# Healthcare-Robotics/assistive-vr-gym

Hardware: AMD Instinct MI355X
Metric: env-steps/sec at N parallel envs, 1/2/4/8 MI355X; max |dq| vs PyBullet (higher is better)
Workload: dtype f32; 1 GPU; FeedingJaco-v0, 4096 envs/GPU, rigid-only, random actions; task=FeedingJaco-v0, envs_per_gpu=4096, impairment=random, parallelism=env-sharded x1, env_groups=4, stepping=rollout

## Files before the change

### assistive-vr-gym_amd/csrc/avr_kernel.hip

```cpp
#include <hip/hip_runtime.h>
#include <stdint.h>

#include "../../include/avr.h"
#include <cstring>
#include <cstdlib>
#include "avr_math.h"

#include "avr_kmodel.h"

typedef float f2v __attribute__((ext_vector_type(2)));
typedef float f4v __attribute__((ext_vector_type(4)));
typedef __attribute__((address_space(3))) float lds_f;
#define AVR_GA __attribute__((address_space(1)))
template <class T> __device__ __forceinline__ T gld(const T *p) { return *(const AVR_GA T *)p; }
__device__ __forceinline__ int2 gld(const int2 *p) { const AVR_GA int *q = (const AVR_GA int *)p; return make_int2(q[0], q[1]); }
__device__ __forceinline__ float2 gld(const float2 *p) { const f2v x = *(const AVR_GA f2v *)p; return make_float2(x.x, x.y); }
__device__ __forceinline__ float4 gld(const float4 *p) { const f4v x = *(const AVR_GA f4v *)p; return make_float4(x.x, x.y, x.z, x.w); }
__device__ __forceinline__ v3 gld3(const float *p) { const AVR_GA float *q = (const AVR_GA float *)p; return V(q[0], q[1], q[2]); }
__device__ __forceinline__ qt gldq(const float *p) { const AVR_GA float *q = (const AVR_GA float *)p; return Q(q[0], q[1], q[2], q[3]); }
__device__ __forceinline__ tf gldtf(const float *p) { tf r; r.p = gld3(p); r.q = gldq(p + 3); return r; }
typedef __attribute__((address_space(3))) f2v lds_f2;
typedef __attribute__((address_space(3))) f4v lds_f4;
typedef __attribute__((address_space(3))) int lds_i;
typedef const __attribute__((address_space(1))) float *gfp;
// ... 3253 lines not shown
    pcount(33, T);
#endif
    for (int c0 = 0; c0 < T; c0 += 64) {
#ifdef AVR_PROF
        int pit = 0, pk = -1;
#endif
        if (c0 + lane < T) {
            float *cs;
            (void)item(c0 + lane, cs);
            const int2 e = entry(c0 + lane);
            const float *bt = btfs[slot_of(c0 + lane)];
            const int k = e.x & 0xffff;
            const int sa = e.y & 0xffff, sb = e.y >> 16;
            const int ba = (e.x >> 16) & 0xff, bb = (e.x >> 24) & 0xff;
            const int vrow = cs_vrow(m, cs), vbo = vrow * m.nb, vso = vrow * m.ns;
            const float thr = fminf(gld(m.body_threshold + (vbo + ba)), gld(m.body_threshold + (vbo + bb)));
            const WShape A = make_wshape(m, sa, ldtf(bt + 8 * ba), vso), B = make_wshape(m, sb, ldtf(bt + 8 * bb), vso);
            int rc = 2;
            v3 nB = V(0, 0, 0), pB = V(0, 0, 0);
            float d = 0.f;
            if (!((A.nv > SMALL_NV && A.tab < 0) || (B.nv > SMALL_NV && B.tab < 0))) {
                int nit, nkind;
                rc = narrowphase<false>(m, *(EpaBuf *)cs, A, B, thr, nB, pB, d, nit, nkind);
#ifdef AVR_PROF
                pit = nit; pk = nkind;
#endif
            }
            np_store(cs, k, rc, nB, pB, d);
        }
#ifdef AVR_PROF
        int mx = pit;
        for (int o = 32; o; o >>= 1) mx = max(mx, __shfl_xor(mx, o));
        int sm = pit;
        for (int o = 32; o; o >>= 1) sm += __shfl_xor(sm, o);
        pcount(36, sm);
        pcount(37, mx);
        pcount(38, __popcll(__ballot(pk == 3)));
        pcount(39, __popcll(__ballot(pk >= 0 && pk < 3)));
#endif
    }
}

__global__ __launch_bounds__(64) __attribute__((amdgpu_waves_per_eu(NP_WAVES))) void avr_narrowphase_kernel(const KModel *__restrict__ mp, const unsigned char *__restrict__ mask, int env0,
                                                             int n_envs) {
    const int list = (blockIdx.x >> 3) & 1;
    const int eb = env0 + 8 * NP_ENVS * (blockIdx.x >> 4) + (blockIdx.x & 7);
    if (eb >= n_envs) return;
    __shared__ float2 ent[NP_ENVS * MAXSP];
    __shared__ float btfs[NP_ENVS][MAXB * 8];
    np_list(*mp, mask, eb, list, n_envs, ent, btfs);
}

#ifndef AVR_COOP_KERNEL
#define AVR_COOP_KERNEL 0
#endif
#if AVR_COOP_KERNEL
__global__ __launch_bounds__(64) void avr_coop_kernel(const KModel *__restrict__ mp, const unsigned char *__restrict__ mask, int env0, int n_envs) {
    __shared__ EpaBuf E;
    AVR_ENV_GUARD();
    if (gld(env_cs(m, env) + CS_COOP) != 0.f) {
        float *ws = env_ws(m, env);
        const int rot = __float_as_int(gld(ws + WS_COOPROT));
        (void)np_coop(m, env_cs(m, env), __float_as_int(gld(env_cs(m, env) + CS_NSP)), E, rot, 1 << 30);
        if (lane_id() == 0) ws[WS_COOPROT] = __int_as_float(rot + AVR_COOP_CAP);
    }
}
#endif

AVR_DI void substep_a_env(const KModel &m, EnvLDS &L, float *__restrict__ state, float dt, int env, int n_envs) {
    (void)n_envs;
    WT_START();
    static_assert(sizeof(EpaBuf) <= sizeof(EnvLDS), "EPA buffer overlay");
#if !AVR_COOP_KERNEL
    float *gst = state + (size_t)env * K_STATE_WORDS;
    const bool persist = gld(gst + S_TASK + T_COOPN) >= (float)AVR_COOP_PERSIST;
    int demand = 0;
    if (gld(env_cs(m, env) + CS_COOP) != 0.f) {
        float *ws = env_ws(m, env);
        const int rot = __float_as_int(gld(ws + WS_COOPROT));
        demand = np_coop(m, env_cs(m, env), __float_as_int(gld(env_cs(m, env) + CS_NSP)), *reinterpret_cast<EpaBuf *>(&L), rot,
                         persist ? AVR_COOP_CAP : 1 << 30);
        if (lane_id() == 0) ws[WS_COOPROT] = __int_as_float(rot + AVR_COOP_CAP);
        SYNC();
    }
#endif
#if AVR_COOP_KERNEL
    float *gst = state + (size_t)env * K_STATE_WORDS;
#endif
    load_a(m, L, gst, env_cs(m, env));
#if !AVR_COOP_KERNEL
    if (lane_id() == 0) {
        L.st[S_TASK + T_COOPN] = demand > AVR_COOP_CAP ? L.st[S_TASK + T_COOPN] + 1.f : 0.f;
        if (persist && demand > AVR_COOP_CAP) L.flags |= 32;
    }
    SYNC();
#endif
    bool ok = substep_a(m, L, dt, gst, env_ws(m, env), env_rows(m, env), env_cs(m, env), K_DYN_ROLE ? env_dynho(m, env) : nullptr);
#ifdef AVR_PROF
    if (lane_id() == 0) env_ws(m, env)[WS_XCC] = __int_as_float(xcc_id());
#endif
    if (lane_id() == 0 && !ok) L.flags |= 1;
    SYNC();
    if (lane_id() == 0) L.st[S_TASK + T_FLAGS] = (float)((int)L.st[S_TASK + T_FLAGS] | L.flags);
    SYNC();
    if (lane_id() < 16) gst[S_TASK + lane_id()] = L.st[S_TASK + lane_id()];
    prof_flush(m, L, env);
    WT_END(0);
}

__global__ __launch_bounds__(64) AVR_KATTR void avr_substep_a_kernel(const KModel *__restrict__ mp, float *__restrict__ state,
                                                                     const unsigned char *__restrict__ mask, float dt, int env0, int n_envs) {
    __shared__ EnvLDS L;
    AVR_ENV_GUARD();
    substep_a_env(m, L, state, dt, env, n_envs);
}

#if B4_PK
struct DV { float rq, rq2; f2v v1, v2, v3; };
#else
struct DV { float rq, rq2, vx, vy, vz, wx, wy, wz; };
#endif

AVR_DI int uni(int x) { return __builtin_amdgcn_readfirstlane(x); }

#define B4_OOB 0x7fff0000
typedef __amdgpu_buffer_rsrc_t rsrc_t;
typedef unsigned u4v __attribute__((ext_vector_type(4)));
typedef unsigned u3v __attribute__((ext_vector_type(3)));
typedef unsigned u2v __attribute__((ext_vector_type(2)));
AVR_DI f4v bld4(rsrc_t r, int o) { u4v x = __builtin_amdgcn_raw_buffer_load_b128(r, o, 0, 0); return *(f4v *)&x; }
AVR_DI f2v bld2(rsrc_t r, int o) { u2v x = __builtin_amdgcn_raw_buffer_load_b64(r, o, 0, 0); return *(f2v *)&x; }
AVR_DI float bld1(rsrc_t r, int o) { return __uint_as_float(__builtin_amdgcn_raw_buffer_load_b32(r, o, 0, 0)); }
#if NDL == 2
typedef f4v rv_t;
#define RVB 16
#define rload bld4
#else
typedef f2v rv_t;
#define RVB 8
#define rload bld2
#endif
typedef __attribute__((address_space(3))) rv_t lds_rv;
AVR_DI f4v bld3(rsrc_t r, int o) {
    u3v x = __builtin_amdgcn_raw_buffer_load_b96(r, o, 0, 0);
    f4v y = {__uint_as_float(x.x), __uint_as_float(x.y), __uint_as_float(x.z), 0.f};
    return y;
}

#ifndef B4_LDSW
#define B4_LDSW 10240
#endif
AVR_DI int al4(int x) { return (x + 3) & ~3; }

AVR_DI int own_of(int mask) {
    const int sl = lane_id() & 15;
    return (int)__builtin_amdgcn_ubfe((unsigned)mask, sl < MAXF ? 2 * sl : 30, 2);
}
static_assert(2 * MAXF <= CI_SLOT && MAXNC + K_CROWS * K_MAX_CONTACTS < (1 << (30 - CI_SLOT)), "own mask and slot bit fields");


struct NcRow { int o; lds_f *ip; f4v h0, h1; float imp; f2v j0, j1, j2; rv_t r; };
struct NcSrc {
    typedef NcRow Row;
    static constexpr bool robot_parts = true;
    rsrc_t rs;
    int eo, ro;
    lds_f *ip0, *nullip;
    AVR_DI void set(Row &R, bool v, int o, lds_f *ip) const { R.o = v ? o : B4_OOB; R.ip = v ? ip : nullip; }
    AVR_DI void hdr(Row &R) const { R.h0 = bld4(rs, R.o); R.h1 = bld3(rs, R.o + 16); R.imp = *R.ip; }
    AVR_DI void parts(Row &R) const {
        const int o = own_of(__float_as_int(R.h0.x));
        const int b = o ? R.o + 8 + 24 * o : B4_OOB;
        R.j0 = bld2(rs, b); R.j1 = bld2(rs, b + 8); R.j2 = bld2(rs, b + 16);
        const int slot = __float_as_int(R.h0.y) - 1;
        R.r = rload(rs, slot >= 0 ? ro + slot * (ROBW * 4) + RVB * (lane_id() & 15) : B4_OOB);
    }
};

#define LN_HEAD (NDL == 2 ? 80 : 48)
#define LNB_NULL 24
#define LNB_ZERO 48
#define LNB_NCNULL 16
typedef __attribute__((address_space(3))) char lds_c;
struct NcLds {
    typedef NcRow Row;
    static constexpr bool robot_parts = true;
    lds_c *blk;
    int eo;
    unsigned rob;
    lds_f *ip0, *nullip;
    AVR_DI void set(Row &R, bool v, int o, lds_f *ip) const { R.o = v ? o : LNB_NCNULL; R.ip = v ? ip : nullip; }
    AVR_DI void hdr(Row &R) const {
        R.h0 = *(const lds_f4 *)(blk + R.o - 8);
        const f2v a = *(const lds_f2 *)(blk + R.o + 8);
        R.h1.x = a.x; R.h1.y = a.y; R.h1.z = *(const lds_f *)(blk + R.o + 16);
        R.imp = *R.ip;
    }
    AVR_DI void parts(Row &R) const {
        const int w = own_of(__float_as_int(R.h0.x));
        const lds_f2 *q = (const lds_f2 *)(blk + (w ? R.o + 24 * w : LNB_ZERO));
        R.j0 = q[0]; R.j1 = q[1]; R.j2 = q[2];
        const unsigned sp = (unsigned)__float_as_int(R.h0.y);
        R.r = *(const lds_rv *)(blk + (sp ? rob + ROBW * 4 * sp : LNB_ZERO));
    }
};

struct CRowL { unsigned wb; lds_f *ip; f4v h; float imp; f2v j0, j1, j2; rv_t r; };
template <bool RC>
struct CLds {
    typedef CRowL Row;
    static constexpr bool robot_parts = RC;
    lds_c *blk;
    unsigned cn, cf;
    unsigned rob;
    lds_f *ipn, *ipf, *nullip;
    unsigned ct;
    lds_f *ipt;
    AVR_DI void set(Row &R, bool v, unsigned wb, lds_f *ip) const { R.wb = v ? wb : LNB_NULL; R.ip = v ? ip : nullip; }
    AVR_DI void hdr(Row &R) const { R.h = *(const lds_f4 *)(blk + R.wb + 8); R.imp = *R.ip; }
    AVR_DI void hdr3(Row &R) const {
        const lds_f *q = (const lds_f *)(blk + R.wb + 8);
        const f2v a = *(const lds_f2 *)q;
        R.h.x = a.x; R.h.y = a.y; R.h.z = q[2];
        R.imp = *R.ip;
    }
    AVR_DI void hdr2(Row &B, const Row &A) const {
        B.h = *(const lds_f4 *)(blk + A.wb + 8 + CRW * 4);
        B.imp = A.ip[1];
    }
    AVR_DI unsigned own_b(const Row &R) const { const int o = own_of(__float_as_int(R.h.x)); return o ? R.wb + 24 * o : LNB_ZERO; }
    AVR_DI void own_at(Row &R, unsigned b) const { const lds_f2 *q = (const lds_f2 *)(blk + b); R.j0 = q[0]; R.j1 = q[1]; R.j2 = q[2]; }
    AVR_DI unsigned rob_b(const Row &R) const { const unsigned s = (unsigned)__float_as_int(R.h.x) >> CI_SLOT; return s ? rob + ROBW * 4 * s : LNB_ZERO; }
    AVR_DI rv_t rob_at(unsigned b) const {
        if constexpr (!RC) { (void)b; return rv_t{}; }
        return *(const lds_rv *)(blk + b);
    }
    AVR_DI void parts(Row &R) const { own_at(R, own_b(R)); R.r = rob_at(rob_b(R)); }
    AVR_DI int tor_of(int c) const { return (int)((unsigned)__float_as_int(*(const lds_f *)(blk + cn + CRW * 4 * c + 8)) >> 2 & 0x3ffffu); }
    AVR_DI void unit_parts(Row &A, Row &B) const {
        const unsigned b = own_b(A), r = rob_b(A);
        own_at(A, b); own_at(B, b + CRW * 4);
        A.r = rob_at(r); B.r = rob_at(r + ROBW * 4);
    }
};

struct CRowG { int o; lds_f *ip; f4v h; float imp; f2v j0, j1, j2; rv_t r; };
struct CGlb {
    typedef CRowG Row;
    static constexpr bool robot_parts = true;
    rsrc_t rs;
    int cn, cf;
    int rob;
    lds_f *ipn, *ipf, *nullip;
    int ct;
    lds_f *ipt;
    AVR_DI void set(Row &R, bool v, int o, lds_f *ip) const { R.o = v ? o : B4_OOB; R.ip = v ? ip : nullip; }
    AVR_DI void hdr(Row &R) const { R.h = bld4(rs, R.o); R.imp = *R.ip; }
    AVR_DI void hdr3(Row &R) const { R.h = bld3(rs, R.o); R.imp = *R.ip; }
    AVR_DI void hdr2(Row &B, const Row &A) const { B.h = bld4(rs, A.o + CRW * 4); B.imp = A.ip[1]; }
    AVR_DI int own_b(const Row &R) const { const int o = own_of(__float_as_int(R.h.x)); return o ? R.o - 8 + 24 * o : B4_OOB; }
    AVR_DI void own_at(Row &R, int b) const { R.j0 = bld2(rs, b); R.j1 = bld2(rs, b + 8); R.j2 = bld2(rs, b + 16); }
    AVR_DI int rob_b(const Row &R) const { const int s = (int)((unsigned)__float_as_int(R.h.x) >> CI_SLOT); return s ? rob + ROBW * 4 * s : B4_OOB; }
    AVR_DI rv_t rob_at(int b) const { return rload(rs, b); }
    AVR_DI void parts(Row &R) const { own_at(R, own_b(R)); R.r = rob_at(rob_b(R)); }
    AVR_DI int tor_of(int c) const { return (int)((unsigned)__float_as_int(bld1(rs, cn + CRW * 4 * c)) >> 2 & 0x3ffffu); }
    AVR_DI void unit_parts(Row &A, Row &B) const {
        const int b = own_b(A), r = rob_b(A);
        own_at(A, b); own_at(B, b + CRW * 4);
        A.r = rob_at(r); B.r = rob_at(r + ROBW * 4);
    }
};

AVR_DI float row16_sum(float x) {
    x += __int_as_float(__builtin_amdgcn_update_dpp(0, __float_as_int(x), 0x128, 0xf, 0xf, true));
    x += __int_as_float(__builtin_amdgcn_update_dpp(0, __float_as_int(x), 0x124, 0xf, 0xf, true));
    x += __int_as_float(__builtin_amdgcn_update_dpp(0, __float_as_int(x), 0x122, 0xf, 0xf, true));
    x += __int_as_float(__builtin_amdgcn_update_dpp(0, __float_as_int(x), 0x121, 0xf, 0xf, true));
    return x;
}

template <bool RP, class R>
AVR_DI float go4(const R &X, DV &d, float imp, float inv, float rhs, float lo, float hi, float rl = 0.f, unsigned long long *acc = nullptr) {
#pragma clang fp contract(off)
#if B4_PK
    f2v s = X.j0 * d.v1;
    if (RP) {
        s.y = fmaf(X.r.x, d.rq, s.y);
#if NDL == 2
        s.y = fmaf(X.r.z, d.rq2, s.y);
#endif
    }
    s = __builtin_elementwise_fma(X.j1, d.v2, s);
    s = __builtin_elementwise_fma(X.j2, d.v3, s);
    const float dv = row16_sum(s.x + s.y);
    const float ni = __builtin_amdgcn_fmed3f(imp + fmaf(-dv, inv, rhs), lo, hi);
    const float delta = ni - imp;
    if (acc) *acc |= __ballot(fabsf(delta) > rl);
    const f2v dd = {delta, delta};
    d.v1 = __builtin_elementwise_fma(X.j0, dd, d.v1);
    d.v2 = __builtin_elementwise_fma(X.j1, dd, d.v2);
    d.v3 = __builtin_elementwise_fma(X.j2, dd, d.v3);
    if (RP) d.rq = fmaf(X.r.y, delta, d.rq);
#if NDL == 2
    if (RP) d.rq2 = fmaf(X.r.w, delta, d.rq2);
#endif
    return ni;
#else
    const float p = fmaf(X.j1.x, d.vz, fmaf(X.j0.y, d.vy, X.j0.x * d.vx));
#if NDL == 2
    const float q = RP ? fmaf(X.j2.y, d.wz, fmaf(X.j2.x, d.wy, fmaf(X.r.z, d.rq2, fmaf(X.r.x, d.rq, X.j1.y * d.wx))))
                       : fmaf(X.j2.y, d.wz, fmaf(X.j2.x, d.wy, X.j1.y * d.wx));
#else
    const float q = RP ? fmaf(X.j2.y, d.wz, fmaf(X.j2.x, d.wy, fmaf(X.r.x, d.rq, X.j1.y * d.wx)))
                       : fmaf(X.j2.y, d.wz, fmaf(X.j2.x, d.wy, X.j1.y * d.wx));
#endif
    const float dv = row16_sum(p + q);
    const float ni = __builtin_amdgcn_fmed3f(imp + fmaf(-dv, inv, rhs), lo, hi);
    const float delta = ni - imp;
    if (acc) *acc |= __ballot(fabsf(delta) > rl);
    d.vx = fmaf(X.j0.x, delta, d.vx); d.vy = fmaf(X.j0.y, delta, d.vy); d.vz = fmaf(X.j1.x, delta, d.vz);
    d.wx = fmaf(X.j1.y, delta, d.wx); d.wy = fmaf(X.j2.x, delta, d.wy); d.wz = fmaf(X.j2.y, delta, d.wz);
    if (RP) d.rq = fmaf(X.r.y, delta, d.rq);
#if NDL == 2
    if (RP) d.rq2 = fmaf(X.r.w, delta, d.rq2);
#endif
    return ni;
#endif
}

#if B4_FPAIR
template <bool RP, class R>
AVR_DI void go4_pair(const R &A, const R &B, DV &d, float &ia, float &ib, float lim) {
#pragma clang fp contract(off)
    f2v sa = A.j0 * d.v1, sb = B.j0 * d.v1;
    if (RP) {
        sa.y = fmaf(A.r.x, d.rq, sa.y); sb.y = fmaf(B.r.x, d.rq, sb.y);
#if NDL == 2
        sa.y = fmaf(A.r.z, d.rq2, sa.y); sb.y = fmaf(B.r.z, d.rq2, sb.y);
#endif
    }
    sa = __builtin_elementwise_fma(A.j1, d.v2, sa); sb = __builtin_elementwise_fma(B.j1, d.v2, sb);
    sa = __builtin_elementwise_fma(A.j2, d.v3, sa); sb = __builtin_elementwise_fma(B.j2, d.v3, sb);
    const float dva = row16_sum(sa.x + sa.y), dvb0 = row16_sum(sb.x + sb.y);
    const float na = __builtin_amdgcn_fmed3f(ia + fmaf(-dva, A.h.y, A.h.z), -lim, lim);
    const float da = na - ia;
    const float dvb = fmaf(da, B.h.w, dvb0);
    const float nb = __builtin_amdgcn_fmed3f(ib + fmaf(-dvb, B.h.y, B.h.z), -lim, lim);
    const float db = nb - ib;
    const f2v dda = {da, da}, ddb = {db, db};
    d.v1 = __builtin_elementwise_fma(B.j0, ddb, __builtin_elementwise_fma(A.j0, dda, d.v1));
    d.v2 = __builtin_elementwise_fma(B.j1, ddb, __builtin_elementwise_fma(A.j1, dda, d.v2));
    d.v3 = __builtin_elementwise_fma(B.j2, ddb, __builtin_elementwise_fma(A.j2, dda, d.v3));
    if (RP) d.rq = fmaf(B.r.y, db, fmaf(A.r.y, da, d.rq));
#if NDL == 2
    if (RP) d.rq2 = fmaf(B.r.w, db, fmaf(A.r.w, da, d.rq2));
#endif
    ia = na; ib = nb;
}
#endif

template <int D, bool H3, class S>
AVR_DI void hdr_of(const S &s, typename S::Row &R) {
    if constexpr (H3) s.hdr3(R);
    else s.hdr(R);
}
template <int D, bool H3, class S, class AT, class GO>
AVR_DI void sweep4(const S &s, int n, const AT &at, const GO &go) {
    if (n <= 0) return;
    constexpr int K = 2 * D + 1;
    typename S::Row R[K];
#pragma unroll
    for (int q = 0; q < 2 * D; q++) { at(R[q], q); hdr_of<D, H3>(s, R[q]); }
#pragma unroll
    for (int q = 0; q < D; q++) s.parts(R[q]);
    for (int j = 0; j < n; j += K) {
#pragma unroll
        for (int q = 0; q < K; q++) {
            at(R[(q + 2 * D) % K], j + q + 2 * D);
            hdr_of<D, H3>(s, R[(q + 2 * D) % K]);
            s.parts(R[(q + D) % K]);
            go(R[q]);
        }
    }
}

template <class S>
struct Pair4 { typename S::Row a, b; float in; };

#if K_TORSION
template <class CS>
struct TorRow : CS::Row { float in; };
template <class CS>
struct TorSrc {
    typedef TorRow<CS> Row;
    static constexpr bool robot_parts = CS::robot_parts;
    const CS &cs;
    AVR_DI void hdr(Row &R) const { cs.hdr(R); }
    AVR_DI void parts(Row &R) const { cs.parts(R); }
};
#endif

AVR_DI int wave_max4(int x) {
    x = max(x, __shfl_xor(x, 16));
    x = max(x, __shfl_xor(x, 32));
    return uni(x);
}

template <int DN, int DC, class NS, class CS>
AVR_DI int pgs4(const KModel &m, const NS &ns, const CS &cs, lds_i *list, lds_i *tlist, int n_nc, int n_c, int nnc_max, int nc_max, DV &d) {
    typedef typename NS::Row NR;
    typedef typename CS::Row CR;
    const int sl = lane_id() & 15;
#if B4_PK
    d.rq = d.rq2 = 0.f; d.v1 = d.v2 = d.v3 = f2v{0.f, 0.f};
#else
    d.rq = d.rq2 = 0.f; d.vx = d.vy = d.vz = d.wx = d.wy = d.wz = 0.f;
#endif
    auto at_n = [&](CR &R, int j) { cs.set(R, j < n_c, cs.cn + CRW * 4 * j, cs.ipn + j); };
    sweep4<DC, true>(cs, nc_max, at_n, [&](const CR &R) { (void)go4<CS::robot_parts>(R, d, 0.f, R.h.y, R.h.z, R.imp, R.imp); });
    int units = 0;
    bool done = false;
    for (int it = 0; it < m.iters; it++) {
        const int a_nc = done ? 0 : n_nc, a_c = done ? 0 : n_c;
        const int anc_max = wave_max4(a_nc), ac_max = wave_max4(a_c);
        unsigned long long acc = 0ull;
        const bool fwd = (it & 1) != 0;
        const int r0 = fwd ? 0 : n_nc - 1, sg = fwd ? 1 : -1;
        const int ob = ns.eo + r0 * (RWC * 4);
        lds_f *ib = ns.ip0 + r0;
        sweep4<DN, false>(ns, anc_max, [&](NR &R, int j) { ns.set(R, j < a_nc, ob + sg * j * (RWC * 4), ib + sg * j); },
                          [&](const NR &R) { *R.ip = go4<true>(R, d, R.imp, R.h0.z, R.h0.w, R.h1.x, R.h1.y, R.h1.z, &acc); });
        auto at_na = [&](CR &R, int j) { cs.set(R, j < a_c, cs.cn + CRW * 4 * j, cs.ipn + j); };
        sweep4<DC, false>(cs, ac_max, at_na, [&](const CR &R) { *R.ip = go4<CS::robot_parts>(R, d, R.imp, R.h.y, R.h.z, 0.f, 1e10f, R.h.w, &acc); });
        int t = 0;
        for (int c0 = 0; c0 < ac_max; c0 += 16) {
            const int c = c0 + sl;
            const bool a = c < a_c && cs.ipn[c < a_c ? c : 0] > 0.f;
            const unsigned long long b = __ballot(a);
            const unsigned gm = (unsigned)(b >> (lane_id() & 48)) & 0xffffu;
            if (a) list[t + __popc(gm & ((1u << sl) - 1u))] = c;
            t += __popc(gm);
        }
        const int tmax = wave_max4(t);
        units += tmax;
        if (tmax > 0) {
        constexpr int K = 2 * DC + 1;
        Pair4<CS> X[K];
        auto lst = [&](int u) { const int c = list[u < t ? u : 0]; return u < t ? c : -1; };
        auto hdr = [&](Pair4<CS> &Y, int c) {
            cs.set(Y.a, c >= 0, cs.cf + 2 * CRW * 4 * c, cs.ipf + 2 * c);
            cs.hdr(Y.a);
            cs.hdr2(Y.b, Y.a);
            const float x = cs.ipn[max(c, 0)];
            Y.in = c >= 0 ? x : 0.f;
        };
        auto go = [&](const Pair4<CS> &Y) {
            const float lim = Y.a.h.w * Y.in;
#if B4_FPAIR
            float ia = Y.a.imp, ib = Y.b.imp;
            go4_pair<CS::robot_parts>(Y.a, Y.b, d, ia, ib, lim);
            Y.a.ip[0] = ia; Y.a.ip[1] = ib;
#else
            Y.a.ip[0] = go4<CS::robot_parts>(Y.a, d, Y.a.imp, Y.a.h.y, Y.a.h.z, -lim, lim, Y.b.h.x, &acc);
            Y.a.ip[1] = go4<CS::robot_parts>(Y.b, d, Y.b.imp, Y.b.h.y, Y.b.h.z, -lim, lim, Y.b.h.w, &acc);
#endif
        };
        int cn = lst(0);
#pragma unroll
        for (int q = 0; q < 2 * DC; q++) { hdr(X[q], cn); cn = lst(q + 1); }
#pragma unroll
        for (int q = 0; q < DC; q++) cs.unit_parts(X[q].a, X[q].b);
        for (int u0 = 0; u0 < tmax; u0 += K) {
#pragma unroll
            for (int q = 0; q < K; q++) {
                hdr(X[(q + 2 * DC) % K], cn);
                cn = lst(u0 + q + 2 * DC + 1);
                cs.unit_parts(X[(q + DC) % K].a, X[(q + DC) % K].b);
                go(X[q]);
            }
        }
#if K_TORSION
        {
            int tt = 0;
            for (int u0 = 0; u0 < tmax; u0 += 16) {
                const int u = u0 + sl;
                const int cl = list[u < t ? u : 0];
                const int c = u < t ? cl : 0;
                const int tv = cs.tor_of(c);
                const bool a = u < t && tv > 0;
                const unsigned long long b = __ballot(a);
                const unsigned gm = (unsigned)(b >> (lane_id() & 48)) & 0xffffu;
                if (a) tlist[tt + __popc(gm & ((1u << sl) - 1u))] = c | (tv - 1) << 8;
                tt += __popc(gm);
            }
            int ttmax = tt;
            ttmax = max(ttmax, __shfl_xor(ttmax, 16));
            ttmax = max(ttmax, __shfl_xor(ttmax, 32));
            ttmax = uni(ttmax);
            const TorSrc<CS> ts{cs};
            sweep4<DC, false>(ts, 3 * ttmax, [&](TorRow<CS> &R, int j) {
                const int u = j / 3, k = j - 3 * u;
                const bool v = u < tt;
                const int e = tlist[v ? u : 0];
                const int c = e & 255, ti = e >> 8;
                cs.set(R, v, cs.ct + 3 * CRW * 4 * ti + CRW * 4 * k, cs.ipt + 3 * ti + k);
                const float x = cs.ipn[v ? c : 0];
                R.in = v ? x : 0.f;
            }, [&](const TorRow<CS> &R) {
                const float lim = R.h.w * R.in;
                *R.ip = go4<CS::robot_parts>(R, d, R.imp, R.h.y, R.h.z, -lim, lim, BT_RESIDUAL_SQRT * R.h.y, &acc);
            });
        }
#endif
        }
        done = done || ((acc >> (lane_id() & 48)) & 0xffffull) == 0ull;
        if (__ballot(!done) == 0ull) break;
    }
    return units;
}

#ifndef B4_DN
#define B4_DN 2
#endif
#ifndef B4_DC
#define B4_DC 1
#endif
#ifndef B4_DG
#define B4_DG 3
#endif
#ifndef B4_NC_LDS
#define B4_NC_LDS K_PR2
#endif
#ifndef B4_DNL
#define B4_DNL 1
#endif

#ifndef B4_SORT
#define B4_SORT 0
#endif
AVR_DI int b4_env(const KModel &m, const unsigned char *__restrict__ mask, int env0, int n_envs, int bidx, int g) {
    const int x = bidx & 7, j = bidx >> 3;
#if B4_SORT
    const int lane = lane_id();
    const int kc = (j >> 5) << 7;
    unsigned key[2];
#pragma unroll
    for (int h = 0; h < 2; h++) {
        const int kk = lane + 64 * h;
        const int e = env0 + x + 8 * (kc + kk);
        unsigned cost = 0xffffffu;
        if (e < n_envs) {
            cost = 0u;
            if (!mask || mask[e]) {
                const float *ws = env_ws(m, e);
                cost = (unsigned)(__float_as_int(gld(ws + WS_NNC)) + 3 * __float_as_int(gld(ws + WS_NC)) +
                                  (K_TORSION ? 3 * __float_as_int(gld(ws + WS_NT)) : 0));
                cost = min(cost, 0xfffffeu);
            }
        }
        key[h] = (cost << 7) | (unsigned)kk;
    }
    int rank0 = 0, rank1 = 0;
    for (int i = 0; i < 64; i++) {
        const unsigned a = __builtin_amdgcn_readlane(key[0], i), b = __builtin_amdgcn_readlane(key[1], i);
        rank0 += (a < key[0]) + (b < key[0]);
        rank1 += (a < key[1]) + (b < key[1]);
    }
    int pick = 0;
#pragma unroll
    for (int gg = 0; gg < 4; gg++) {
        const int r = 4 * (j & 31) + gg;
        const unsigned long long b0 = __ballot(rank0 == r), b1 = __ballot(rank1 == r);
        const int kk = b0 ? __builtin_ctzll(b0) : 64 + __builtin_ctzll(b1);
        if (g == gg) pick = kk;
    }
    return env0 + x + 8 * (kc + pick);
#else
    (void)m; (void)mask; (void)n_envs;
    return env0 + 32 * j + x + 8 * g;
#endif
}

AVR_DI void substep_b4_block(const KModel &m, float *__restrict__ state, const unsigned char *__restrict__ mask, float dt, int frame_end,
                             int env0, int n_envs, int bidx, lds_f *blk) {
#ifdef AVR_WAVETIME
    const unsigned long long wt0 = __builtin_amdgcn_s_memrealtime();
#endif
    const int lane = lane_id(), sl = lane & 15, g = lane >> 4;
    const int env = b4_env(m, mask, env0, n_envs, bidx, g);
    const bool live = env < n_envs && (!mask || mask[env]);
    const int ev = live ? env : env0;
    const gfp wsg = (gfp)env_ws(m, ev);
    float *st = state + (size_t)ev * K_STATE_WORDS;
    const int n_nc = live ? __float_as_int(wsg[WS_NNC]) : 0, n_c = live ? __float_as_int(wsg[WS_NC]) : 0;
    const int n_rob = live ? __float_as_int(wsg[WS_NROB]) : 0;
    const int n_t = live && K_TORSION ? __float_as_int(wsg[WS_NT]) : 0;
    const int n_cr = 3 * n_c + 3 * n_t;
    const int n_rows = n_nc + n_cr, n_rc = max(n_rob - n_nc, 0);
    auto wmax = [&](int x) { x = max(x, __shfl_xor(x, 16)); x = max(x, __shfl_xor(x, 32)); return uni(x); };
    const int nnc_max = wmax(n_nc), nc_max = wmax(n_c);
    const rsrc_t rs = __builtin_amdgcn_make_buffer_rsrc(m.rows, 0, m.rows_envs * m.rowstride * 4, 0x00020000);
    const int eo = ev * m.rowstride * 4, ro = eo + m.rowcap * RWC * 4;
#ifdef AVR_LDS_POISON
    for (int i = lane; i < B4_LDSW; i += 64) blk[i] = __int_as_float(-1);
    SYNC();
#endif
    const int szA = al4(n_rows + 2) + (K_TORSION ? 2 : 1) * al4(n_c), szB = n_cr * CRW + n_rc * ROBW;
#if B4_NC_LDS
    const int szF = szB + n_nc * (RWC + ROBW);
    const int f0 = __shfl(szA + szF, 0), f1 = __shfl(szA + szF, 16), f2 = __shfl(szA + szF, 32), f3 = __shfl(szA + szF, 48);
    const bool full = uni(f0 + f1 + f2 + f3) <= B4_LDSW - LN_HEAD && !m.b4_global;
#else
    const int f0 = 0, f1 = 0, f2 = 0;
    constexpr bool full = false;
#endif
    const int t0 = __shfl(szA + szB, 0), t1 = __shfl(szA + szB, 16), t2 = __shfl(szA + szB, 32), t3 = __shfl(szA + szB, 48);
    const bool in_lds = full || (uni(t0 + t1 + t2 + t3) <= B4_LDSW - LN_HEAD && !m.b4_global);
    int base;
    if (full) base = g == 0 ? 0 : g == 1 ? f0 : g == 2 ? f0 + f1 : f0 + f1 + f2;
    else if (in_lds) base = g == 0 ? 0 : g == 1 ? t0 : g == 2 ? t0 + t1 : t0 + t1 + t2;
    else {
        const int a0 = __shfl(szA, 0), a1 = __shfl(szA, 16), a2 = __shfl(szA, 32);
        base = g == 0 ? 0 : g == 1 ? a0 : g == 2 ? a0 + a1 : a0 + a1 + a2;
    }
    base += LN_HEAD;
    lds_f *imp = blk + base;
    lds_i *list = (lds_i *)(imp + al4(n_rows + 2));
    lds_i *tlist = list + al4(n_c);
    const int cw = base + szA, nw = cw + n_cr * CRW, rw = full ? nw + n_nc * RWC : nw;
    const gfp cpool = (gfp)(st + S_CP);
    float wimp[K_MAX_CONTACTS / 16];
#pragma unroll
    for (int q = 0; q < K_MAX_CONTACTS / 16; q++) wimp[q] = cpool[AVR_CP_WORDS * min(sl + 16 * q, max(n_c - 1, 0)) + AVR_CP_IMP];
    for (int r = sl; r < n_rows + 2; r += 16) {
        const int c = r - n_nc;
        if (!(c >= 0 && c < n_c)) imp[r] = 0.f;
    }
    for (int i = lane; i < LN_HEAD; i += 64) blk[i] = 0.f;
    if (in_lds) {
        const int n4r = n_cr * (CRW / 4), n4n = full ? n_nc * (RWC / 4) : 0, n4s = (full ? n_rob : n_rc) * (ROBW / 4);
        const int n4a = n4r + n4n, n4 = n4a + n4s, so = full ? ro : ro + n_nc * ROBW * 4;
        const int m4 = wmax(n4);
        lds_f4 *l0 = (lds_f4 *)(blk + cw);
        for (int b = 0; b < m4; b += 8 * 16) {
            f4v t[8];
#pragma unroll
            for (int q = 0; q < 8; q++) {
                const int i = b + 16 * q + sl;
                t[q] = bld4(rs, i < n4r ? eo + CR_BASE * 4 + 16 * i : i < n4a ? eo + 16 * (i - n4r) : (i < n4 ? so + 16 * (i - n4a) : B4_OOB));
            }
#pragma unroll
            for (int q = 0; q < 8; q++) {
                const int i = b + 16 * q + sl;
                if (i < n4) l0[i] = t[q];
            }
        }
    }
#pragma unroll
    for (int q = 0; q < K_MAX_CONTACTS / 16; q++)
        if (sl + 16 * q < n_c) imp[n_nc + sl + 16 * q] = wimp[q] * m.warmstart;
    SYNC();
    lds_f *const ipn = imp + n_nc, *const ipf = ipn + n_c, *const ipt = ipf + 2 * n_c, *const nullip = imp + n_rows;
    NcSrc ns{rs, eo, ro, imp, nullip};
    DV d;
    int units, rcb = 0;
#if B4_NC_LDS
    if (full) {
        const unsigned cn = 4 * cw - 8, cf = cn + 4 * CRW * n_c, ct = cf + 8 * CRW * n_c, rob = 4 * (rw - ROBW) + RVB * sl;
        const NcLds nl{(lds_c *)blk, 4 * nw + 8, rob, imp, nullip};
        if (wmax(n_rc) > 0) {
            CLds<true> cs{(lds_c *)blk, cn, cf, rob, ipn, ipf, nullip, ct, ipt};
            units = pgs4<B4_DNL, B4_DC>(m, nl, cs, list, tlist, n_nc, n_c, nnc_max, nc_max, d);
            rcb = 1;
        } else {
            CLds<false> cs{(lds_c *)blk, cn, cf, rob, ipn, ipf, nullip, ct, ipt};
            units = pgs4<B4_DNL, B4_DC>(m, nl, cs, list, tlist, n_nc, n_c, nnc_max, nc_max, d);
        }
    } else
#endif
    if (in_lds) {
        const unsigned cn = 4 * cw - 8, cf = cn + 4 * CRW * n_c, ct = cf + 8 * CRW * n_c, rob = 4 * (rw - (n_nc + 1) * ROBW) + RVB * sl;
        if (wmax(n_rc) > 0) {
            CLds<true> cs{(lds_c *)blk, cn, cf, rob, ipn, ipf, nullip, ct, ipt};
            units = pgs4<B4_DN, B4_DC>(m, ns, cs, list, tlist, n_nc, n_c, nnc_max, nc_max, d);
            rcb = 1;
        } else {
            CLds<false> cs{(lds_c *)blk, cn, cf, rob, ipn, ipf, nullip, ct, ipt};
            units = pgs4<B4_DN, B4_DC>(m, ns, cs, list, tlist, n_nc, n_c, nnc_max, nc_max, d);
        }
    } else {
        const int cn = eo + CR_BASE * 4, cf = cn + 4 * CRW * n_c, ct = cf + 8 * CRW * n_c, rob = ro - ROBW * 4 + RVB * sl;
        CGlb cs{rs, cn, cf, rob, ipn, ipf, nullip, ct, ipt};
        units = pgs4<B4_DN, B4_DG>(m, ns, cs, list, tlist, n_nc, n_c, nnc_max, nc_max, d);
    }
    (void)units; (void)rcb;
    for (int c = sl; c < n_c; c += 16) st[S_CP + AVR_CP_WORDS * c + AVR_CP_IMP] = imp[n_nc + c];
#ifdef AVR_WAVETIME
    {
        const unsigned long long wt1 = __builtin_amdgcn_s_memrealtime();
        const int e0 = env0 + 32 * (bidx >> 3) + (bidx & 7);
        if (m.prof && lane == 0 && e0 < n_envs) {
            m.prof[((size_t)1 * n_envs + e0) * 2] = wt0;
            m.prof[((size_t)1 * n_envs + e0) * 2 + 1] = wt1;
            m.prof[((size_t)2 * n_envs + e0) * 2] = (unsigned long long)nnc_max | (unsigned long long)nc_max << 16 | (unsigned long long)in_lds << 32;
            m.prof[((size_t)2 * n_envs + e0) * 2 + 1] = (unsigned long long)wmax(n_rows) | (unsigned long long)units << 16 | (unsigned long long)rcb << 40 | (unsigned long long)xcc_id() << 44;
        }
    }
#endif
    if (!live) return;
    const float *ws = env_ws(m, ev);
#if B4_PK
    struct { float vx, vy, vz, wx, wy, wz; } dl = {d.v1.x, d.v2.x, d.v3.x, d.v1.y, d.v2.y, d.v3.y};
#else
    DV &dl = d;
#endif
    if (sl < m.nf) {
        const qt q = ldq(st + S_FREE + AVR_FB_WORDS * sl + 3);
        const v3 I = gld3(m.fb_inertia + 4 * sl);
        const float rs = 1.f / sqrtf(gld(m.fb_mass + (sl)));
        const v3 sd = V(sqrtf(I.x > 0.f ? 1.f / I.x : 0.f), sqrtf(I.y > 0.f ? 1.f / I.y : 0.f), sqrtf(I.z > 0.f ? 1.f / I.z : 0.f));
        const v3 w = qrot(q, V(dl.wx * sd.x, dl.wy * sd.y, dl.wz * sd.z));
        dl.vx *= rs; dl.vy *= rs; dl.vz *= rs;
        dl.wx = w.x; dl.wy = w.y; dl.wz = w.z;
    }
    const float vmax = m.max_vel;
    const int nda = env_hdyn(m, st) ? m.nd + m.hc_n : m.nd;
#pragma unroll
    for (int k = 0; k < NDL; k++) {
        const int dof = sl + 16 * k;
        if (dof < nda) {
            float v = clampf(ws[WS_VQ + dof] + (k == 0 ? d.rq : d.rq2), -vmax, vmax);
            float q = st[S_Q + dof] + dt * v;
            if (frame_end && dof >= m.nd) {
#if K_CHAIN_LIMITS_IN_STATE
                const float lo = st[S_HCH + 2 * K_HC_N + (dof - m.nd)], hi = st[S_HCH + 3 * K_HC_N + (dof - m.nd)];
#else
                const float lo = gld(m.hc_lower + (dof - m.nd)), hi = gld(m.hc_upper + (dof - m.nd));
#endif
                if (q < lo) { q = lo; v = 0.f; }
                else if (q > hi) { q = hi; v = 0.f; }
            }
            st[S_QD + dof] = v;
            st[S_Q + dof] = q;
        }
    }
    if (sl < m.nf) {
        float *fb = st + S_FREE + AVR_FB_WORDS * sl;
        v3 v = clamp3(add(ld3(ws + WS_FV + 4 * sl), V(dl.vx, dl.vy, dl.vz)), vmax);
        v3 om = clamp3(add(ld3(ws + WS_FW + 4 * sl), V(dl.wx, dl.wy, dl.wz)), vmax);
        st3(fb + 7, v);
        st3(fb + 10, om);
        st3(fb, add(ld3(fb), scl(v, dt)));
        float ang = len(om);
        if (ang * dt > BT_ANGULAR_MOTION_THRESHOLD) ang = (0.5f * 1.5707963267948966f) / dt;
        v3 ax;
        if (ang < 0.001f) ax = scl(om, 0.5f * dt - (dt * dt * dt) * 0.020833333333f * ang * ang);
        else ax = scl(om, sinf(0.5f * ang * dt) / ang);
        qt dq = Q(ax.x, ax.y, ax.z, cosf(ang * dt * 0.5f));
        stq(fb + 3, qnorm(qmul(dq, ldq(fb + 3))));
    }
}

__global__ __launch_bounds__(64) void avr_substep_b4_kernel(const KModel *__restrict__ mp, float *__restrict__ state,
                                                            const unsigned char *__restrict__ mask, float dt, int frame_end, int env0,
                                                            int n_envs) {
    __shared__ f4v b4l[B4_LDSW / 4];
    substep_b4_block(*mp, state, mask, dt, frame_end, env0, n_envs, blockIdx.x, (lds_f *)(lds_f4 *)b4l);
}



#if AVR_TASK == AVR_TASK_FEEDING
__global__ __launch_bounds__(64) void avr_task_kernel(const KModel *__restrict__ mp, float *__restrict__ state, float *__restrict__ obs,
                                                      float *__restrict__ rew, unsigned char *__restrict__ done, float *__restrict__ info,
                                                      const unsigned char *__restrict__ mask, int mode, int env0, int n_envs) {
    __shared__ EnvLDS L;
    AVR_ENV_GUARD();
    const int lane = lane_id();
    float *gst = state + (size_t)env * K_STATE_WORDS;
    const float *gcp = gst + S_CP;
    load_state(m, L, gst);
    PROF_START(ptask);
    if (L.nla > m.nl) robot_fk(m, L);
    mouth_target(m, L);
    if (mode == MODE_SETTLE) {
        if (obs) observe(m, L, 0.f, obs + (size_t)env * K_OBS_DIM);
    } else if (mode == MODE_STEP || mode == MODE_STEP_RANDOM) {
        if (lane == 0) L.st[S_TASK + T_ITER] += 1.f;
        SYNC();
        int dummy;
        float robot_force = contact_sum(m, L, gcp, 0, 0, 0, dummy);
        float spoon_force = contact_sum(m, L, gcp, 1, 0, 0, dummy);
        float food_reward = 0.f, hit_reward = 0.f, mouth_vel = 0.f;
        int alive = (int)L.st[S_TASK + T_ALIVE], hit = (int)L.st[S_TASK + T_HIT];
        float succ = L.st[S_TASK + T_SUCCESS];
        v3 tgt = ld3(L.st + S_TASK + T_TARGET);
        for (int k = 0; k < m.n_food; k++) {
            if (!(alive >> k & 1)) continue;
            float *fb = L.st + S_FREE + AVR_FB_WORDS * (m.food_free0 + k);
            v3 fp = ld3(fb);
            int fbody = m.food_body0 + k;
            if (len(sub(tgt, fp)) < 0.02f) {
                food_reward += 20.f;
                succ += 1.f;
                mouth_vel += len(ld3(fb + 7));
                alive &= ~(1 << k);
                SYNC();
                if (lane == 0) st3(fb, V(1500.f + 10.f * k, 1500.f, 1500.f));
                SYNC();
                continue;
            }
            int ctab, cbowl, chum;
            contact_sum(m, L, gcp, 2, fbody, m.table_body, ctab);
            contact_sum(m, L, gcp, 2, fbody, m.bowl_body, cbowl);
            if (fp.z < 0.5f || ctab > 0 || cbowl > 0) {
                food_reward -= 5.f;
                alive &= ~(1 << k);
                continue;
            }
            contact_sum(m, L, gcp, 3, fbody, 0, chum);
            if (chum > 0 && !(hit >> k & 1)) { hit |= 1 << k; hit_reward -= 1.f; }
        }
        SYNC();
        if (lane == 0) {
            L.st[S_TASK + T_ALIVE] = (float)alive;
            L.st[S_TASK + T_HIT] = (float)hit;
            L.st[S_TASK + T_SUCCESS] = succ;
        }
        SYNC();
        const float *sp = L.st + S_FREE + AVR_FB_WORDS * m.spoon_free;
        float ee_vel = len(ld3(sp + 7));
        observe(m, L, spoon_force, obs + (size_t)env * K_OBS_DIM);
        float prefs = m.w_velocity * (-ee_vel) + m.w_force_nontarget * (-robot_force) +
                      m.w_high_forces * (spoon_force < 10.f ? 0.f : -spoon_force) + m.w_food_hit * hit_reward +
                      m.w_food_velocities * (-mouth_vel);
        float dist = len(sub(tgt, ld3(sp)));
        float asq = env_ws(m, env)[WS_ASQ];
        float r = m.w_distance * (-dist) + m.w_action * (-asq) + m.w_food * food_reward + prefs;
        if (lane == 0) {
            rew[env] = r;
            int itn = (int)L.st[S_TASK + T_ITER];
            done[env] = (unsigned char)(itn >= m.max_steps);
            info[(size_t)env * AVR_INFO_DIM + 0] = robot_force + spoon_force;
            info[(size_t)env * AVR_INFO_DIM + 1] = succ >= (float)m.n_food * m.task_success_threshold ? 1.f : 0.f;
        }
    }
    SYNC();
    bool bad = false;
    for (int i = lane; i < S_CP; i += 64) bad |= !(L.st[i] == L.st[i]);
// ... 230 lines not shown
```

Baseline: 940,500 env-steps/s.

## Precompute packed LDS addresses and interleave impulses in triplets for PGS sweeps

When the contact data lives in LDS, the solver's row lists now store packed LDS byte offsets for the header and the impulse slot instead of contact indices. The normal, friction and torsion impulses are interleaved in groups of three, and zeroed guard rows are added so out-of-range lanes clamp to a valid null row instead of using select logic. This removes per-row index-to-address arithmetic and conditional selects from the inner sweep loops. In exchange it changes the LDS layout and footprint, which can affect when environments fit in LDS, and adds complexity to the packing of the 16-bit address fields.

After: 967,600 env-steps/s (median of 6 runs). 1.03x the previous value.

```diff
diff --git a/assistive-vr-gym_amd/csrc/avr_kernel.hip b/assistive-vr-gym_amd/csrc/avr_kernel.hip
--- a/assistive-vr-gym_amd/csrc/avr_kernel.hip
+++ b/assistive-vr-gym_amd/csrc/avr_kernel.hip
@@ -3429,6 +3429,13 @@
 #endif
 AVR_DI int al4(int x) { return (x + 3) & ~3; }
 
+#ifndef B4_ADDR
+#define B4_ADDR 1
+#endif
+#define B4_NP (B4_ADDR && B4_NC_LDS ? 1 : 0)
+AVR_DI unsigned lds_addr(const __attribute__((address_space(3))) void *p) { return (unsigned)(size_t)p; }
+AVR_DI __attribute__((address_space(3))) float *lds_at(unsigned a) { return (__attribute__((address_space(3))) float *)(size_t)a; }
+
 AVR_DI int own_of(int mask) {
     const int sl = lane_id() & 15;
     return (int)__builtin_amdgcn_ubfe((unsigned)mask, sl < MAXF ? 2 * sl : 30, 2);
@@ -3439,7 +3446,7 @@
 struct NcRow { int o; lds_f *ip; f4v h0, h1; float imp; f2v j0, j1, j2; rv_t r; };
 struct NcSrc {
     typedef NcRow Row;
-    static constexpr bool robot_parts = true;
+    static constexpr bool robot_parts = true, addr = false;
     rsrc_t rs;
     int eo, ro;
     lds_f *ip0, *nullip;
@@ -3461,7 +3468,7 @@
 typedef __attribute__((address_space(3))) char lds_c;
 struct NcLds {
     typedef NcRow Row;
-    static constexpr bool robot_parts = true;
+    static constexpr bool robot_parts = true, addr = B4_ADDR != 0;
     lds_c *blk;
     int eo;
     unsigned rob;
@@ -3486,7 +3493,7 @@
 template <bool RC>
 struct CLds {
     typedef CRowL Row;
-    static constexpr bool robot_parts = RC;
+    static constexpr bool robot_parts = RC, addr = B4_ADDR != 0;
     lds_c *blk;
     unsigned cn, cf;
     unsigned rob;
@@ -3524,7 +3531,7 @@
 struct CRowG { int o; lds_f *ip; f4v h; float imp; f2v j0, j1, j2; rv_t r; };
 struct CGlb {
     typedef CRowG Row;
-    static constexpr bool robot_parts = true;
+    static constexpr bool robot_parts = true, addr = false;
     rsrc_t rs;
     int cn, cf;
     int rob;
@@ -3693,7 +3700,13 @@
 #else
     d.rq = d.rq2 = 0.f; d.vx = d.vy = d.vz = d.wx = d.wy = d.wz = 0.f;
 #endif
-    auto at_n = [&](CR &R, int j) { cs.set(R, j < n_c, cs.cn + CRW * 4 * j, cs.ipn + j); };
+    auto at_n = [&](CR &R, int j) {
+        if constexpr (CS::addr) {
+            const unsigned k = (unsigned)min(j, n_c);
+            R.wb = cs.cn + CRW * 4 * k;
+            R.ip = (lds_f *)((lds_c *)cs.ipn + __umul24(k, 12u));
+        } else cs.set(R, j < n_c, cs.cn + CRW * 4 * j, cs.ipn + j);
+    };
     sweep4<DC, true>(cs, nc_max, at_n, [&](const CR &R) { (void)go4<CS::robot_parts>(R, d, 0.f, R.h.y, R.h.z, R.imp, R.imp); });
     int units = 0;
     bool done = false;
@@ -3705,31 +3718,61 @@
         const int r0 = fwd ? 0 : n_nc - 1, sg = fwd ? 1 : -1;
         const int ob = ns.eo + r0 * (RWC * 4);
         lds_f *ib = ns.ip0 + r0;
-        sweep4<DN, false>(ns, anc_max, [&](NR &R, int j) { ns.set(R, j < a_nc, ob + sg * j * (RWC * 4), ib + sg * j); },
+        const int no = fwd ? n_nc - a_nc : a_nc - 1;
+        sweep4<DN, false>(ns, anc_max, [&](NR &R, int j) {
+                              if constexpr (NS::addr) {
+                                  const unsigned k = min((unsigned)(no + sg * j), (unsigned)n_nc);
+                                  R.o = ns.eo + (int)__umul24(k, (unsigned)(RWC * 4));
+                                  R.ip = ns.ip0 + k;
+                              } else ns.set(R, j < a_nc, ob + sg * j * (RWC * 4), ib + sg * j);
+                          },
                           [&](const NR &R) { *R.ip = go4<true>(R, d, R.imp, R.h0.z, R.h0.w, R.h1.x, R.h1.y, R.h1.z, &acc); });
-        auto at_na = [&](CR &R, int j) { cs.set(R, j < a_c, cs.cn + CRW * 4 * j, cs.ipn + j); };
+        unsigned nb = cs.cn + CRW * 4 * (n_c - a_c);
+        lds_c *const nib = (lds_c *)cs.ipn + 12 * (n_c - a_c);
+        if constexpr (CS::addr) asm("" : "+v"(nb));
+        auto at_na = [&](CR &R, int j) {
+            if constexpr (CS::addr) {
+                const unsigned k = (unsigned)min(j, a_c);
+                R.wb = nb + CRW * 4 * k;
+                R.ip = (lds_f *)(nib + __umul24(k, 12u));
+            } else cs.set(R, j < a_c, cs.cn + CRW * 4 * j, cs.ipn + j);
+        };
         sweep4<DC, false>(cs, ac_max, at_na, [&](const CR &R) { *R.ip = go4<CS::robot_parts>(R, d, R.imp, R.h.y, R.h.z, 0.f, 1e10f, R.h.w, &acc); });
         int t = 0;
         for (int c0 = 0; c0 < ac_max; c0 += 16) {
             const int c = c0 + sl;
-            const bool a = c < a_c && cs.ipn[c < a_c ? c : 0] > 0.f;
+            const bool a = c < a_c && cs.ipn[(CS::addr ? 3 : 1) * (c < a_c ? c : 0)] > 0.f;
             const unsigned long long b = __ballot(a);
             const unsigned gm = (unsigned)(b >> (lane_id() & 48)) & 0xffffu;
-            if (a) list[t + __popc(gm & ((1u << sl) - 1u))] = c;
+            if constexpr (CS::addr) {
+                if (a) list[t + __popc(gm & ((1u << sl) - 1u))] = (int)((cs.cf + 2 * CRW * 4 * c) | lds_addr(cs.ipf + 3 * c) << 16);
+            } else if (a) list[t + __popc(gm & ((1u << sl) - 1u))] = c;
             t += __popc(gm);
         }
+        if constexpr (CS::addr) list[t] = (int)((unsigned)LNB_NULL | lds_addr(cs.nullip) << 16);
         const int tmax = wave_max4(t);
         units += tmax;
         if (tmax > 0) {
         constexpr int K = 2 * DC + 1;
         Pair4<CS> X[K];
-        auto lst = [&](int u) { const int c = list[u < t ? u : 0]; return u < t ? c : -1; };
+        auto lst = [&](int u) {
+            if constexpr (CS::addr) return list[min(u, t)];
+            else { const int c = list[u < t ? u : 0]; return u < t ? c : -1; }
+        };
         auto hdr = [&](Pair4<CS> &Y, int c) {
-            cs.set(Y.a, c >= 0, cs.cf + 2 * CRW * 4 * c, cs.ipf + 2 * c);
-            cs.hdr(Y.a);
-            cs.hdr2(Y.b, Y.a);
-            const float x = cs.ipn[max(c, 0)];
-            Y.in = c >= 0 ? x : 0.f;
+            if constexpr (CS::addr) {
+                Y.a.wb = (unsigned)c & 0xffffu;
+                Y.a.ip = lds_at((unsigned)c >> 16);
+                cs.hdr(Y.a);
+                cs.hdr2(Y.b, Y.a);
+                Y.in = Y.a.ip[2];
+            } else {
+                cs.set(Y.a, c >= 0, cs.cf + 2 * CRW * 4 * c, cs.ipf + 2 * c);
+                cs.hdr(Y.a);
+                cs.hdr2(Y.b, Y.a);
+                const float x = cs.ipn[max(c, 0)];
+                Y.in = c >= 0 ? x : 0.f;
+            }
         };
         auto go = [&](const Pair4<CS> &Y) {
             const float lim = Y.a.h.w * Y.in;
@@ -3757,7 +3800,41 @@
             }
         }
 #if K_TORSION
-        {
+        if constexpr (CS::addr) {
+            typedef __attribute__((address_space(3))) u2v lds_u2;
+            lds_u2 *const tl = (lds_u2 *)tlist;
+            int tt = 0;
+            for (int u0 = 0; u0 < tmax; u0 += 16) {
+                const int u = u0 + sl;
+                const unsigned e = (unsigned)list[min(u, t)];
+                const int c = u < t ? (int)((e & 0xffffu) - cs.cf) >> 7 : 0;
+                const int tv = cs.tor_of(c);
+                const float in = lds_at(e >> 16)[2];
+                const bool a = u < t && tv > 0;
+                const unsigned long long b = __ballot(a);
+                const unsigned gm = (unsigned)(b >> (lane_id() & 48)) & 0xffffu;
+                if (a) {
+                    lds_u2 *const q = tl + 3 * (tt + __popc(gm & ((1u << sl) - 1u)));
+                    const unsigned w = (cs.ct + 3 * CRW * 4 * (tv - 1)) | lds_addr(cs.ipt + 3 * (tv - 1)) << 16;
+#pragma unroll
+                    for (int k = 0; k < 3; k++) q[k] = u2v{w + k * (CRW * 4 + (4 << 16)), (unsigned)__float_as_int(in)};
+                }
+                tt += __popc(gm);
+            }
+            const int tr = 3 * tt;
+            tl[tr] = u2v{(unsigned)LNB_NULL | lds_addr(cs.nullip) << 16, 0u};
+            const int ttmax = wave_max4(tt);
+            const TorSrc<CS> ts{cs};
+            sweep4<DC, false>(ts, 3 * ttmax, [&](TorRow<CS> &R, int j) {
+                const u2v e = tl[min(j, tr)];
+                R.wb = e.x & 0xffffu;
+                R.ip = lds_at(e.x >> 16);
+                R.in = __uint_as_float(e.y);
+            }, [&](const TorRow<CS> &R) {
+                const float lim = R.h.w * R.in;
+                *R.ip = go4<CS::robot_parts>(R, d, R.imp, R.h.y, R.h.z, -lim, lim, BT_RESIDUAL_SQRT * R.h.y, &acc);
+            });
+        } else {
             int tt = 0;
             for (int u0 = 0; u0 < tmax; u0 += 16) {
                 const int u = u0 + sl;
@@ -3882,9 +3959,17 @@
     for (int i = lane; i < B4_LDSW; i += 64) blk[i] = __int_as_float(-1);
     SYNC();
 #endif
-    const int szA = al4(n_rows + 2) + (K_TORSION ? 2 : 1) * al4(n_c), szB = n_cr * CRW + n_rc * ROBW;
+#if B4_ADDR
+    constexpr int GN = 4, GNC = 8;
+    const int n_imp = n_rows + 3 + B4_NP;
+    const int szA = al4(n_imp) + al4(n_c + 1) + (K_TORSION ? al4(6 * n_t + 2) : 0), szB = n_cr * CRW + n_rc * ROBW + GN;
+#else
+    constexpr int GN = 0, GNC = 0;
+    const int n_imp = n_rows + 2;
+    const int szA = al4(n_imp) + (K_TORSION ? 2 : 1) * al4(n_c), szB = n_cr * CRW + n_rc * ROBW;
+#endif
 #if B4_NC_LDS
-    const int szF = szB + n_nc * (RWC + ROBW);
+    const int szF = szB + n_nc * (RWC + ROBW) + GNC;
     const int f0 = __shfl(szA + szF, 0), f1 = __shfl(szA + szF, 16), f2 = __shfl(szA + szF, 32), f3 = __shfl(szA + szF, 48);
     const bool full = uni(f0 + f1 + f2 + f3) <= B4_LDSW - LN_HEAD && !m.b4_global;
 #else
@@ -3902,16 +3987,22 @@
     }
     base += LN_HEAD;
     lds_f *imp = blk + base;
-    lds_i *list = (lds_i *)(imp + al4(n_rows + 2));
-    lds_i *tlist = list + al4(n_c);
-    const int cw = base + szA, nw = cw + n_cr * CRW, rw = full ? nw + n_nc * RWC : nw;
+    lds_i *list = (lds_i *)(imp + al4(n_imp));
+    lds_i *tlist = list + al4(n_c + (B4_ADDR ? 1 : 0));
+    const int cw = base + szA, nw = cw + n_cr * CRW + GN, rw = full ? nw + n_nc * RWC + GNC : nw;
+    const bool trip = B4_ADDR && in_lds;
+    const int ins = trip ? 3 : 1;
+    lds_f *const ipt = trip ? imp + n_nc + B4_NP : imp + n_nc + 3 * n_c;
+    lds_f *const ipf = trip ? ipt + 3 * n_t : imp + n_nc + n_c;
+    lds_f *const ipn = trip ? ipf + 2 : imp + n_nc;
+    lds_f *const nullip = trip ? ipf + 3 * n_c : imp + n_rows;
     const gfp cpool = (gfp)(st + S_CP);
     float wimp[K_MAX_CONTACTS / 16];
 #pragma unroll
     for (int q = 0; q < K_MAX_CONTACTS / 16; q++) wimp[q] = cpool[AVR_CP_WORDS * min(sl + 16 * q, max(n_c - 1, 0)) + AVR_CP_IMP];
-    for (int r = sl; r < n_rows + 2; r += 16) {
-        const int c = r - n_nc;
-        if (!(c >= 0 && c < n_c)) imp[r] = 0.f;
+    for (int r = sl; r < n_imp; r += 16) {
+        const int c = r - (int)(ipn - imp);
+        if (!(c >= 0 && c < ins * n_c && (!trip || c % 3 == 0))) imp[r] = 0.f;
     }
     for (int i = lane; i < LN_HEAD; i += 64) blk[i] = 0.f;
     if (in_lds) {
@@ -3929,21 +4020,28 @@
 #pragma unroll
             for (int q = 0; q < 8; q++) {
                 const int i = b + 16 * q + sl;
+#if B4_ADDR
+                if (i < n4) l0[i + (i >= 4 * n_c ? GN / 4 : 0) + (full && i >= n4a ? GNC / 4 : 0)] = t[q];
+#else
                 if (i < n4) l0[i] = t[q];
-            }
-        }
+#endif
+            }
+        }
+#if B4_ADDR
+        if (sl == 0) l0[4 * n_c] = f4v{0.f, 0.f, 0.f, 0.f};
+        if (full && sl < GNC / 4) l0[n4a + GN / 4 + sl] = f4v{0.f, 0.f, 0.f, 0.f};
+#endif
     }
 #pragma unroll
     for (int q = 0; q < K_MAX_CONTACTS / 16; q++)
-        if (sl + 16 * q < n_c) imp[n_nc + sl + 16 * q] = wimp[q] * m.warmstart;
-    SYNC();
-    lds_f *const ipn = imp + n_nc, *const ipf = ipn + n_c, *const ipt = ipf + 2 * n_c, *const nullip = imp + n_rows;
+        if (sl + 16 * q < n_c) ipn[ins * (sl + 16 * q)] = wimp[q] * m.warmstart;
+    SYNC();
     NcSrc ns{rs, eo, ro, imp, nullip};
     DV d;
     int units, rcb = 0;
 #if B4_NC_LDS
     if (full) {
-        const unsigned cn = 4 * cw - 8, cf = cn + 4 * CRW * n_c, ct = cf + 8 * CRW * n_c, rob = 4 * (rw - ROBW) + RVB * sl;
+        const unsigned cn = 4 * cw - 8, cf = cn + 4 * CRW * n_c + 4 * GN, ct = cf + 8 * CRW * n_c, rob = 4 * (rw - ROBW) + RVB * sl;
         const NcLds nl{(lds_c *)blk, 4 * nw + 8, rob, imp, nullip};
         if (wmax(n_rc) > 0) {
             CLds<true> cs{(lds_c *)blk, cn, cf, rob, ipn, ipf, nullip, ct, ipt};
@@ -3956,7 +4054,7 @@
     } else
 #endif
     if (in_lds) {
-        const unsigned cn = 4 * cw - 8, cf = cn + 4 * CRW * n_c, ct = cf + 8 * CRW * n_c, rob = 4 * (rw - (n_nc + 1) * ROBW) + RVB * sl;
+        const unsigned cn = 4 * cw - 8, cf = cn + 4 * CRW * n_c + 4 * GN, ct = cf + 8 * CRW * n_c, rob = 4 * (rw - (n_nc + 1) * ROBW) + RVB * sl;
         if (wmax(n_rc) > 0) {
             CLds<true> cs{(lds_c *)blk, cn, cf, rob, ipn, ipf, nullip, ct, ipt};
             units = pgs4<B4_DN, B4_DC>(m, ns, cs, list, tlist, n_nc, n_c, nnc_max, nc_max, d);
@@ -3971,7 +4069,7 @@
         units = pgs4<B4_DN, B4_DG>(m, ns, cs, list, tlist, n_nc, n_c, nnc_max, nc_max, d);
     }
     (void)units; (void)rcb;
-    for (int c = sl; c < n_c; c += 16) st[S_CP + AVR_CP_WORDS * c + AVR_CP_IMP] = imp[n_nc + c];
+    for (int c = sl; c < n_c; c += 16) st[S_CP + AVR_CP_WORDS * c + AVR_CP_IMP] = ipn[ins * c];
 #ifdef AVR_WAVETIME
     {
         const unsigned long long wt1 = __builtin_amdgcn_s_memrealtime();
```
